# bramtoula/multi_robot_SLAM_separators

Measured on AMD Instinct MI355X. Metric: candidate keyframe-pair verifications/sec (NetVLAD NN + ORB match + RANSAC) @1/2/4/8 GPU, higher is better.
Workload: dtype u8+f16+f32+f64

## Files before the change

### multi_robot_slam_separators_amd/csrc/k_ba.hip

```cpp
#pragma once
#include "sf_device_math.hpp"
#include "sf_internal.hpp"
#include "sf_pnp_math.hpp"

namespace {

#define BA_NSUM 28

struct BaLds {
  double* X;
  double* Xc;
  float* o1;
  float* o2;
  double* red;
  double* ne_a;
  double* ne_b;
  int* misc;
};

struct BaCam {
  double fx, fy, b, info, delta;
  double R1[9], t1[3];
};

// ... 303 lines not shown
      for (int k = 0; k < 3; ++k) tt[k] = c == 0 ? cam.t1[k] : t[k];
      const double* Xi = L.X + 3 * i;
      const double Pc[3] = {((R[0] * Xi[0] + R[1] * Xi[1]) + R[2] * Xi[2]) + tt[0],
                            ((R[3] * Xi[0] + R[4] * Xi[1]) + R[5] * Xi[2]) + tt[1],
                            ((R[6] * Xi[0] + R[7] * Xi[1]) + R[8] * Xi[2]) + tt[2]};
      double r[3], J[3][3];
      const int rows = ba_edge(cam, Pc, (c == 0 ? L.o1 : L.o2) + 3 * i, r, J);
      if (rows == 0) { bad = true; continue; }
      double chi2 = r[0] * r[0] + r[1] * r[1];
      if (rows == 3) chi2 = chi2 + r[2] * r[2];
      chi2 = chi2 * cam.info;
      if (chi2 > lim) bad = true;
    }
    n_out += bad ? 1 : 0;
  }
#pragma unroll
  for (int off = 32; off >= 1; off >>= 1) n_out += __shfl_xor(n_out, off);
  __syncthreads();
  if (lane == 0) L.misc[8 + wave] = n_out;
  __syncthreads();
  n_out = L.misc[8];
#pragma unroll
  for (int w = 1; w < NW; ++w) n_out += L.misc[8 + w];

  if (tid == 0) {
    PassState o = p0;
    o.inliers = n - n_out;
    if (o.inliers < P.min_inliers) {
      o.is_null = 1;
#pragma unroll
      for (int i = 0; i < 12; ++i) o.T[i] = 0.f;
    } else {
// ... 191 lines not shown
#pragma unroll
    for (int w = 0; w < SF_BLOCK / 64; ++w) {
      const int cw = misc[4 + w];
      if (w < wave) woff += cw;
      total += cw;
    }
    if (ok) {
      const int k = n_ba + woff + before;
      pts[k] = make_float4(ax, ay, az, 0.f);
      cidx[k] = c;
      ones[k] = 1;
    }
    n_ba += total;
    __syncthreads();
  }
#pragma unroll
  for (int off = 32; off >= 1; off >>= 1) { uni += __shfl_xor(uni, off); uni_m += __shfl_xor(uni_m, off); }
  if (lane == 0) { atomicAdd(&misc[0], uni); atomicAdd(&misc[1], uni_m); }
  __syncthreads();
  uni = misc[0];
  uni_m = misc[1];
  if (tid == 0) {
    PassState a = fwd[pair];
    const PassState b = back[pair];
    a.matches = PNP ? uni_m : (a.matches > b.matches ? a.matches : b.matches);
    const bool adjust = P.bundle_adjustment != 0 && !a.is_null && n_ba > 0;
    misc[2] = adjust ? 1 : 0;
    if (adjust) {
      a.inliers = n_ba;
    } else {
      a.inliers = uni;
      if (!b.is_null) {
// ... 58 lines not shown
```

### multi_robot_slam_separators_amd/csrc/k_guided.hip

```cpp
#include "sf_device_math.hpp"
#include "sf_internal.hpp"

namespace {

#define GUIDED_CPT 8
#define GUIDED_CAND_CAP (GUIDED_CPT * 256)
#define GUIDED_CAND_CAP_NARROW 1216


__device__ __forceinline__ bool guided_eligible(const PassState& p1, const DeviceParams& P, const int4& mF, int Kf, int Kt,
                                                PassState& pass2_out, uint8_t& guided_flag_out, CorrHeader& hdr_out) {
  bool ident = true;
#pragma unroll
  for (int i = 0; i < 12; ++i) ident = ident && (p1.T[i] == ((i == 0 || i == 5 || i == 10) ? 1.f : 0.f));
  const bool eligible = !p1.is_null && !ident && P.guess_win > 0 && mF.y > 0 && P.calibrated && Kf > 0 && Kt > 0;
  if (!eligible && threadIdx.x == 0) {
    pass2_out = p1;
    guided_flag_out = 0;
    CorrHeader h = {0, 0, 0, 0};
    hdr_out = h;
  }
  return eligible;
}

// ... 54 lines not shown
    __syncthreads();
    int woff = 0, total = 0;
#pragma unroll
    for (int w = 0; w < NW; ++w) {
      int c = misc[4 + w];
      if (w < wave) woff += c;
      total += c;
    }
    if (flag) out[running + woff + before] = (uint32_t)i | ((uint32_t)m << 16);
    running += total;
    __syncthreads();
  }
  return running;
}

__device__ __forceinline__ void guided_sum_counts(int& n_finite, int& n_proj, int* misc) {
  for (int off = 32; off >= 1; off >>= 1) {
    n_finite += __shfl_xor(n_finite, off);
    n_proj += __shfl_xor(n_proj, off);
  }
  if ((threadIdx.x & 63) == 0) {
    atomicAdd(&misc[0], n_finite);
    atomicAdd(&misc[1], n_proj);
  }
  __syncthreads();
  n_finite = misc[0];
  n_proj = misc[1];
}

template <int NW>
__device__ __forceinline__ bool guided_finish(const StoreView& st, int pair, int sT, const int4& mT, int Kt,
                                              const float* xF, int n_finite, int n_proj, int n_corr, const uint32_t* out,
                                              PassState& pass2_out, uint8_t& guided_flag_out, CorrHeader& hdr_out,
                                              int32_t* __restrict__ list, int32_t* __restrict__ counter,
// ... 132 lines not shown
    for (int j = 0; j < 2; ++j) {
      const int t = base + tid + j * NT;
      if (t < Kt) {
        raw[t] = k2[j];
        const int cidx = cell_of(k2[j]);
        if (cidx >= 0) atomicAdd(&cell_start[cidx + 1], 1);
      }
    }
  }
  __syncthreads();
  {
    const int per = (NC + NT - 1) / NT;
    const int c0 = tid * per, c1 = min(c0 + per, NC);
    int local = 0;
    for (int cidx = c0; cidx < c1; ++cidx) local += cell_start[cidx + 1];
    int incl = local;
    for (int off = 1; off < 64; off <<= 1) {
      const int o = __shfl_up(incl, off);
      if (lane >= off) incl += o;
    }
    if (lane == 63) misc[8 + wave] = incl;
    __syncthreads();
    int woff = 0;
    for (int w = 0; w < wave; ++w) woff += misc[8 + w];
    int run = woff + incl - local;
    __syncthreads();
    for (int cidx = c0; cidx < c1; ++cidx) {
      const int cnt_c = cell_start[cidx + 1];
      cell_start[cidx + 1] = run + cnt_c;
      run += cnt_c;
    }
  }
  __syncthreads();
  for (int t = tid; t < Kt; t += NT) {
    const float4 k = raw[t];
// ... 76 lines not shown
                nb = 0;
              }
              const uint32_t rec = ((uint32_t)i << 16) | (uint32_t)t;
              hb0 = nb == 0 ? rec : hb0; hb1 = nb == 1 ? rec : hb1; hb2 = nb == 2 ? rec : hb2; hb3 = nb == 3 ? rec : hb3;
              ++nb;
              ++oi;
              if (last < 0 || t > last) last = t;
            }
          }
        }
      }
    }
#ifdef SF_CHAIN_TRACE
    if (base == 0 && wave == 0 && P.dbg_trace) {
      int mx = dbg_trips, sm = dbg_entries;
      for (int off = 32; off >= 1; off >>= 1) { mx = max(mx, __shfl_xor(mx, off)); sm += __shfl_xor(sm, off); }
      if (lane == 0) P.dbg_trace[(size_t)pair * SF_TRACE_SLOTS + 31] = ((unsigned long long)mx << 32) | (unsigned)sm;
    }
#endif
    if (base == 0) SF_TRACE_MARK(P, pair, 29);
    {
      int incl = nb;
#pragma unroll
      for (int off = 1; off < 64; off <<= 1) {
        const int o = __shfl_up(incl, off);
        if (lane >= off) incl += o;
      }
      const int wtot = __shfl(incl, 63);
      int wbase = 0;
      if (wtot > 0) {
        if (lane == 0) wbase = atomicAdd(&misc[3], wtot);
        wbase = __shfl(wbase, 0);
        const int s0 = wbase + incl - nb;
        if (s0 + nb <= cand_cap) {
          if (nb > 0) cand[s0] = hb0;
          if (nb > 1) cand[s0 + 1] = hb1;
          if (nb > 2) cand[s0 + 2] = hb2;
          if (nb > 3) cand[s0 + 3] = hb3;
        }
      }
    }
    if (base == 0) SF_TRACE_MARK(P, pair, 30);
#ifndef SF_CHAIN_TRACE
// ... 6 lines not shown
    }
#endif
    if (i < Kf) {
      oilast[i] = ((uint32_t)min(oi, 0xFFFF) << 16) | (uint32_t)(last & 0xFFFF);
      key1[i] = 0xFFFFFFFFu;
      key2[i] = 0xFFFFFFFFu;
    }
  }
  __syncthreads();
  SF_TRACE_MARK(P, pair, 24);
  const int n_cand = misc[3];
#ifndef SF_CHAIN_TRACE
  if (P.dbg_trace) {
    int mine = 0;
    for (int i = tid; i < Kf; i += NT) mine += (int)(oilast[i] >> 16);
    for (int off = 32; off >= 1; off >>= 1) mine += __shfl_xor(mine, off);
    if (lane == 0) atomicAdd(&misc[12], mine);
    __syncthreads();
    if (tid == 0 && misc[12] != n_cand) atomicAdd(&P.dbg_trace[2], 1ull);
    __syncthreads();
  }
#endif
#ifdef SF_CHAIN_TRACE
  if (tid == 0 && P.dbg_trace) P.dbg_trace[(size_t)pair * SF_TRACE_SLOTS + 27] = (unsigned long long)n_cand;
#endif
  if (!L2 && n_cand <= cand_cap) {
    if constexpr (NW == 4) {
    uint32_t ck[GUIDED_CPT], ci[GUIDED_CPT];
#pragma unroll
    for (int j = 0; j < GUIDED_CPT; ++j) {
      const int c = tid + j * NT;
// ... 304 lines not shown
          b0 = min(b0, key);
        }
        ++oi;
        one = i;
      }
    }
    int m = -1;
    if (oi >= 2) {
      if constexpr (L2) { if (i0 >= 0 && f0 < P.nndr * f1) m = i0; }
      else if ((float)(b0 >> 16) < P.nndr * (float)(b1 >> 16)) m = (int)(b0 & 0xFFFFu);
    } else if (oi == 1) {
      m = one;
    }
    if (m >= 0 && atomicCAS(&claimw[m], EMPTY, (uint32_t)t) != EMPTY) atomicOr(&claimw[m], SHARED);
  }
  guided_sum_counts(n_finite, n_proj, misc);
  const int n_corr = guided_compact<NW>(Kf, out, misc, [&](int i) {
    const uint32_t w = claimw[i];
    return (w & SHARED) ? -1 : (int)w;
  });
  return guided_finish<NW>(st, pair, sT, mT, Kt, xF, n_finite, n_proj, n_corr, out, pass2_out, guided_flag_out, hdr_out,
                           list, counter, P, misc);
}

template <int W, bool L2 = false>
__global__ void __launch_bounds__(SF_BLOCK)
k_guided_tp(StoreView st, const int32_t* __restrict__ pair_from, const int32_t* __restrict__ pair_to,
            const PassState* __restrict__ pass1, PassState* __restrict__ pass2, uint8_t* __restrict__ guided_flag,
            uint32_t* __restrict__ corr, CorrHeader* __restrict__ hdr, int32_t* __restrict__ list,
            int32_t* __restrict__ counter, DeviceParams P) {
  extern __shared__ __attribute__((aligned(16))) int smem[];
// ... 162 lines not shown
```

### multi_robot_slam_separators_amd/csrc/k_pnp.hip

```cpp
#include "sf_device_math.hpp"
#include "sf_internal.hpp"
#include "sf_pnp_math.hpp"
#include "k_ba.hip"

namespace {

#define PNP_NSUM 28

__host__ __device__ inline size_t sf_pnp_lds_bytes_dev(int kcap, int iterations, bool bear = true, int nw = 4) {
  (void)iterations;
  return (size_t)kcap * (16 + (bear ? 24 : 0) + 8 + 4 + 4 + 4 + 2) + 128 * 8 + 64 * 4 + 16 * 4 + 12 * 64 * 4 +
         (size_t)(nw + 1) * 64 * 4 + 16 * 4 + 2 * 32 * 8;
}

struct PnpLds {
  float4* obj;
  float2* img;
  double* bear;
  uint32_t* cidx;
  float* e1;
  float* e2;
  uint8_t* mask;
  uint8_t* mask_b;
  int* counts;
  double* red;
  int* misc;
  float* hyp;
  int* hyp_cnt;
  float* best;
  double* ne_a;
  double* ne_b;
};

template <int NW = 4>
__device__ __forceinline__ int block_sum_i(int v, int* misc, int tid) {
  const int lane = tid & 63, wave = tid >> 6;
#pragma unroll
  for (int off = 32; off >= 1; off >>= 1) v += __shfl_xor(v, off);
  __syncthreads();
  if (lane == 0) misc[8 + wave] = v;
  __syncthreads();
  int t = misc[8];
#pragma unroll
  for (int w = 1; w < NW; ++w) t += misc[8 + w];
  return t;
}

struct PnpCam {
  double fx, fy;
  float fxf, fyf, thr2f;
};

__device__ __forceinline__ bool pnp_inlier(const PnpLds& L, const PnpCam& cam, const float (&c)[12], int i) {
// ... 33 lines not shown
      const double inv = 1.0 / sqrt((un * un + vn * vn) + 1.0);
      f[k][0] = un * inv; f[k][1] = vn * inv; f[k][2] = inv;
    }
  }
  const float4 p4 = L.obj[s3];
  const float2 o4 = L.img[s3];
  const double P4[3] = {(double)p4.x, (double)p4.y, (double)p4.z};
  return sfd::p3p_best(P, f, P4, (double)o4.x, (double)o4.y, cam.fx, cam.fy, coef);
}

template <int NW>
__device__ inline void pnp_normal_eq(const PnpLds& L, const PnpCam& cam, int m, const uint8_t* mask,
                                     const double (&q)[4], const double (&t)[3], double* out, int tid) {
  double R[9];
  sfd::quat_to_R(q, R);
  sfd::canon_reduce_to_lds<PNP_NSUM, 32, NW>(m, tid, L.red, out, [&](int i, double (&ne)[PNP_NSUM]) {
    if (!mask[i]) return;
    const float4 p = L.obj[i];
    const float2 o = L.img[i];
    const double Px = (double)p.x, Py = (double)p.y, Pz = (double)p.z;
    const double Yx = (R[0] * Px + R[1] * Py) + R[2] * Pz;
    const double Yy = (R[3] * Px + R[4] * Py) + R[5] * Pz;
    const double Yz = (R[6] * Px + R[7] * Py) + R[8] * Pz;
    const double X = Yx + t[0], Y = Yy + t[1], Z = Yz + t[2];
    if (Z > 0.0) {
      const double iz = 1.0 / Z;
      const double xn = X * iz, yn = Y * iz;
      const double ru = cam.fx * xn - (double)o.x;
      const double rv = cam.fy * yn - (double)o.y;
      const double a0 = cam.fx * iz, a2 = -(a0 * xn);
      const double b1 = cam.fy * iz, b2 = -(b1 * yn);
// ... 382 lines not shown
    int n_sizes = 0, z1 = 0, z2 = 0, z3 = 0, z4 = 0;
    do {
      pnp_lm<NW>(L, cam, m, prev, q, t, tid);
      z4 = z3; z3 = z2; z2 = z1; z1 = n_prev;
      ++n_sizes;
      __syncthreads();
      n_new = pnp_select<NW>(L, cam, m, q, t, error_threshold, neu, tid);
      if (n_new < min_count) {
        ++refine_iterations;
        if (refine_iterations >= P.pnp_refine_iterations) break;
        continue;
      }
      double s1[1] = {0.0};
      if constexpr (NW == 4) {
        for (int i = tid; i < m; i += NT) if (neu[i]) s1[0] += (double)L.e1[i];
        sfd::block_sum_canon<1, 32>(s1, L.red, tid);
      } else {
        sfd::canon_reduce<1, 32, NW>(m, tid, L.red, s1, [&](int i, double (&a)[1]) { if (neu[i]) a[0] += (double)L.e1[i]; });
      }
      const float mean = (float)(s1[0] / (double)n_new);
      float variance = 0.0f;
      if (n_new > 1) {
        double s2[1] = {0.0};
        if constexpr (NW == 4) {
          for (int i = tid; i < m; i += NT) {
            if (neu[i]) { const float dlt = L.e1[i] - mean; s2[0] += (double)(dlt * dlt); }
          }
          sfd::block_sum_canon<1, 32>(s2, L.red, tid);
        } else {
          sfd::canon_reduce<1, 32, NW>(m, tid, L.red, s2, [&](int i, double (&a)[1]) {
            if (neu[i]) { const float dlt = L.e1[i] - mean; a[0] += (double)(dlt * dlt); }
          });
        }
        variance = (float)(s2[0] / (double)(n_new - 1));
      }
      const float sthr = (float)P.refine_sigma * sqrtf(variance);
      error_threshold = sthr < inlier_thr ? sthr : inlier_thr;
      inlier_changed = false;
      { uint8_t* tp = prev; prev = neu; neu = tp; const int tn = n_prev; n_prev = n_new; n_new = tn; }
      if (n_new != n_prev) {
        if (n_sizes >= 4 && z1 == z3 && z2 == z4) break;
        inlier_changed = true;
        continue;
// ... 122 lines not shown
  const bool guided = guided_flag != nullptr && guided_flag[pair] != 0;
  const bool g0 = sf_pnp_dir_gate(0, h, st.meta[sF].x, guided, min_inliers);
  const bool g1 = sf_pnp_dir_gate(1, h, st.meta[sF].x, guided, min_inliers);
  const float* xF = st.xyz + (size_t)sF * kcap * 3;
  const float* xT = st.xyz + (size_t)sT * kcap * 3;
  const uint32_t* cl = corr + (size_t)pair * kcap;
  int uni = 0, uni_m = 0;
  for (int i = lane; i < kcap; i += 64) uni += (mask_f[(size_t)pair * kcap + i] | mask_b[(size_t)pair * kcap + i]) ? 1 : 0;
  for (int i = lane; i < h.n_corr; i += 64) {
    const uint32_t c = cl[i];
    bool m = false;
    if (g0) { const float* a = xF + 3 * (c & 0xFFFFu); m = sfd::finite3(a[0], a[1], a[2]); }
    if (g1 && !m) { const float* b = xT + 3 * (c >> 16); m = sfd::finite3(b[0], b[1], b[2]); }
    uni_m += m ? 1 : 0;
  }
#pragma unroll
  for (int off = 32; off >= 1; off >>= 1) { uni += __shfl_xor(uni, off); uni_m += __shfl_xor(uni_m, off); }
  if (lane != 0) return;
  PassState a = fwd[pair];
  const PassState b = back[pair];
  a.inliers = uni;
  a.matches = uni_m;
  if (!b.is_null) {
    float inv[12];
    sfd::rigid_inverse_canon(b.T, inv);
    if (a.is_null) {
#pragma unroll
      for (int i = 0; i < 12; ++i) a.T[i] = inv[i];
      a.is_null = 0;
      a.var = b.var;
      a.var_ang = b.var_ang;
    } else {
// ... 78 lines not shown
```

### multi_robot_slam_separators_amd/csrc/k_ransac.hip

```cpp
#include "sf_device_math.hpp"
#include "sf_internal.hpp"
#include "k_ba.hip"

namespace {

struct RansacLds {
  float4* src;
  float4* dst;
  float* d2;
  uint8_t* mask_a;
  uint8_t* mask_b;
  double* red;
  unsigned long long* sums;
  int* misc;
  float* hyp;
  int* hyp_cnt;
  float* best;
  float* bc;
  uint32_t* cidx;
};

__device__ __forceinline__ RansacLds ransac_carve(unsigned char* p, int kcap) {
  RansacLds L;
  L.src = (float4*)p; p += (size_t)kcap * 16;
// ... 113 lines not shown
  for (int i = tid; i < m4; i += 64 * NW) {
    float r2 = __int_as_float(0x7F800000);
    if (i < m) {
      float4 p = L.src[i], q = L.dst[i];
      const float v = sfd::residual2(coef, p.x, p.y, p.z, q.x, q.y, q.z);
      const bool in = (double)v < thr2;
      r2 = in ? v : r2;
      const bool was = prev ? prev[i] != 0 : false;
      mask[i] = in ? 1 : 0;
      const bool low = in && !(thr < sigma * sqrt(2.1981 * (double)v));
      acc += (in ? 1ull : 0ull) + (low ? (1ull << 13) : 0ull) + ((was != in) ? (1ull << 26) : 0ull);
    }
    L.d2[i] = r2;
  }
  const int lane = tid & 63, wave = tid >> 6;
#pragma unroll
  for (int off = 32; off >= 1; off >>= 1) acc += __shfl_xor(acc, off);
  __syncthreads();
  if (lane == 0) L.sums[wave] = acc;
  __syncthreads();
  unsigned long long t = L.sums[0];
#pragma unroll
  for (int w = 1; w < NW; ++w) t += L.sums[w];
  SelCounts c;
  c.n = (int)(t & 0x1FFFull);
  c.low = (int)((t >> 13) & 0x1FFFull);
  c.diff = (int)((t >> 26) & 0x1FFFull);
  return c;
}

typedef __attribute__((address_space(3))) const float* lds_cfloat_p;
typedef __attribute__((address_space(3))) unsigned* lds_uint_p;
// ... 6 lines not shown
  __syncthreads();
  unsigned prefix = 0u;
#pragma unroll 1
  for (int p = 0; p < 4; ++p) {
    const int shift = 24 - 8 * p;
    for (int i = tid; i < m4; i += NT) {
      const unsigned bits = __float_as_uint(d2[i]);
      if (p == 0 || (bits >> (shift + 8)) == prefix)
        __hip_atomic_fetch_add(&hist[p * 256 + ((bits >> shift) & 255u)], 1u, __ATOMIC_RELAXED, __HIP_MEMORY_SCOPE_WORKGROUP);
    }
    __syncthreads();
    if (wave == 0) {
      const unsigned h0 = hist[p * 256 + 4 * lane], h1 = hist[p * 256 + 4 * lane + 1], h2 = hist[p * 256 + 4 * lane + 2],
                     h3 = hist[p * 256 + 4 * lane + 3];
      const unsigned s = (h0 + h1) + (h2 + h3);
      unsigned incl = s;
#pragma unroll
      for (int off = 1; off < 64; off <<= 1) {
        const unsigned y = __shfl_up(incl, off);
        if (lane >= off) incl += y;
      }
      const unsigned excl = incl - s;
      if (excl <= (unsigned)rank && (unsigned)rank < incl) {
        unsigned r = (unsigned)rank - excl;
        int b = 0;
        if (r >= h0) { r -= h0; b = 1; if (r >= h1) { r -= h1; b = 2; if (r >= h2) { r -= h2; b = 3; } } }
        misc[2] = (int)((prefix << 8) | (unsigned)(4 * lane + b));
        misc[3] = (int)r;
      }
    }
    __syncthreads();
    prefix = (unsigned)misc[2];
    rank = misc[3];
  }
  return __uint_as_float(prefix);
}
// ... 49 lines not shown
  if (i < m) {
    const float4 p = L.src[i], q = L.dst[i];
    const float r2 = sfd::residual2(coef, p.x, p.y, p.z, q.x, q.y, q.z);
    cnt += (r2 <= thr2f) ? 1 : 0;
  }
  return cnt;
}

struct ScanState {
  int best;
  int best_it;
  int it;
  double k;
};

__device__ __forceinline__ int shfl_up_from(int v, int off, int lane) {
  const int src = lane >= off ? lane - off : lane;
  return __builtin_amdgcn_ds_bpermute(src << 2, v);
}
__device__ __forceinline__ double shfl_up_from(double v, int off, int lane) {
  const int src = lane >= off ? lane - off : lane;
  const long long b = __double_as_longlong(v);
  const int lo = __builtin_amdgcn_ds_bpermute(src << 2, (int)(b & 0xFFFFFFFFll));
  const int hi = __builtin_amdgcn_ds_bpermute(src << 2, (int)(b >> 32));
  return __longlong_as_double(((long long)hi << 32) | (unsigned)lo);
}

__device__ __forceinline__ bool replay_round(const RansacLds& L, ScanState& S, int base, int R, int lane, int c,
                                             bool present, int max_it, bool adaptive, double inv_m,
                                             double log_probability, bool park = true) {
  int x = present ? c : -1;
#pragma unroll
  for (int off = 1; off < 64; off <<= 1) {
    const int y = shfl_up_from(x, off, lane);
    if (lane >= off) x = max(x, y);
  }
  x = max(x, S.best);
  double kj = 1.0;
  if (x >= 0) {
    const double w = (double)x * inv_m;
    double pno = 1.0 - (w * w) * w;
    if (pno < 2.220446049250313e-16) pno = 2.220446049250313e-16;
    if (pno > 1.0 - 2.220446049250313e-16) pno = 1.0 - 2.220446049250313e-16;
    kj = log_probability / sfd::canon_log(pno);
  }
  double kprev = shfl_up_from(kj, 1, lane);
  if (lane == 0) kprev = S.k;
  const int it = base + lane;
  const bool top_ok = present && (!adaptive || (double)it < kprev) && c >= 0;
  const unsigned long long fail = ~__ballot(top_ok);
  const int n_proc = fail ? (__ffsll((long long)fail) - 1) : 64;
// ... 376 lines not shown
  extern __shared__ __attribute__((aligned(16))) unsigned char smem_raw[];
  const int pair = list[blockIdx.x];
  ransac_body<DIR>(st, pair, pair_from[pair], pair_to[pair], corr + (size_t)pair * st.kcap, hdr[pair].n_corr,
                       pass[pair], P, smem_raw, 2, mask ? mask + (size_t)pair * st.kcap : nullptr);
  if (extra_3dof && threadIdx.x == 0) pass_to3dof(pass[pair], extra_3dof);
}

__global__ void __launch_bounds__(64)
k_merge_directions(const int32_t* __restrict__ list, const int32_t* __restrict__ counter, PassState* __restrict__ fwd,
                   const PassState* __restrict__ back, const uint8_t* __restrict__ mask_f,
                   const uint8_t* __restrict__ mask_b, int kcap, int extra_3dof) {
  if ((int)blockIdx.x >= *counter) return;
  const int pair = list[blockIdx.x], lane = threadIdx.x;
  int uni = 0;
  for (int i = lane; i < kcap; i += 64) uni += (mask_f[(size_t)pair * kcap + i] | mask_b[(size_t)pair * kcap + i]) ? 1 : 0;
#pragma unroll
  for (int off = 32; off >= 1; off >>= 1) uni += __shfl_xor(uni, off);
  if (lane != 0) return;
  PassState a = fwd[pair];
  const PassState b = back[pair];
  a.inliers = uni;
  a.matches = a.matches > b.matches ? a.matches : b.matches;
  if (!b.is_null) {
    float inv[12];
    sfd::rigid_inverse_canon(b.T, inv);
    if (a.is_null) {
#pragma unroll
      for (int i = 0; i < 12; ++i) a.T[i] = inv[i];
      a.is_null = 0;
      a.var = b.var;
      a.var_ang = b.var_ang;
    } else {
// ... 77 lines not shown
```

### multi_robot_slam_separators_amd/csrc/sf_device_math.hpp

```cpp
#pragma once
#include <hip/hip_runtime.h>
#include <stdint.h>

namespace sfd {

__device__ __forceinline__ uint64_t mix64(uint64_t z) {
  z += 0x9E3779B97F4A7C15ULL;
  z = (z ^ (z >> 30)) * 0xBF58476D1CE4E5B9ULL;
  z = (z ^ (z >> 27)) * 0x94D049BB133111EBULL;
  return z ^ (z >> 31);
}

__device__ __forceinline__ void sample_triplet(uint64_t seed, uint32_t it, uint32_t attempt, uint32_t m,
                                               uint32_t& i0, uint32_t& i1, uint32_t& i2) {
  uint64_t ha = mix64(seed ^ mix64(((uint64_t)it << 32) | (uint64_t)attempt));
  uint64_t hb = mix64(ha);
  uint32_t r0 = (uint32_t)(ha >> 32), r1 = (uint32_t)ha, r2 = (uint32_t)(hb >> 32);
  i0 = __umulhi(r0, m);
  i1 = __umulhi(r1, m - 1);
  if (i1 >= i0) ++i1;
  i2 = __umulhi(r2, m - 2);
  uint32_t lo = i0 < i1 ? i0 : i1, hi = i0 < i1 ? i1 : i0;
  if (i2 >= lo) ++i2;
  if (i2 >= hi) ++i2;
// ... 198 lines not shown
    coef[4 * j + 2] = (float)R[3 * j + 2];
    coef[4 * j + 3] = (float)t;
  }
}

__device__ __forceinline__ float residual2(const float (&c)[12], float px, float py, float pz,
                                           float qx, float qy, float qz) {
  float tx = __fmaf_rn(c[2], pz, __fmaf_rn(c[1], py, __fmaf_rn(c[0], px, c[3])));
  float ty = __fmaf_rn(c[6], pz, __fmaf_rn(c[5], py, __fmaf_rn(c[4], px, c[7])));
  float tz = __fmaf_rn(c[10], pz, __fmaf_rn(c[9], py, __fmaf_rn(c[8], px, c[11])));
  float dx = tx - qx, dy = ty - qy, dz = tz - qz;
  return __fmaf_rn(dz, dz, __fmaf_rn(dy, dy, dx * dx));
}


template <int C>
__device__ __forceinline__ void sum_stage(double (&w)[32], int& idx, int lane, int off) {
  if constexpr (C > 1) {
    const bool up = (lane & off) != 0;
#pragma unroll
    for (int k = 0; k < C / 2; ++k) {
      const double send = up ? w[k] : w[k + C / 2];
      const double keep = up ? w[k + C / 2] : w[k];
      w[k] = keep + __shfl_xor(send, off);
    }
    idx += up ? C / 2 : 0;
  } else {
    w[0] = w[0] + __shfl_xor(w[0], off);
  }
}

template <int N, int STRIDE>
__device__ __forceinline__ void block_sum_canon(double (&v)[N], double* red, int tid) {
  static_assert(N >= 1 && N <= 32 && STRIDE >= N, "at most 32 values");
  constexpr int P = N <= 1 ? 1 : N <= 2 ? 2 : N <= 4 ? 4 : N <= 8 ? 8 : N <= 16 ? 16 : 32;
  static_assert(STRIDE >= P, "scratch rows must hold the padded count");
  const int lane = tid & 63, wave = tid >> 6;
  double w[32];
#pragma unroll
  for (int k = 0; k < 32; ++k) w[k] = k < N ? v[k] : 0.0;
  int idx = 0;
  sum_stage<P>(w, idx, lane, 32);
  sum_stage<(P / 2 > 1 ? P / 2 : 1)>(w, idx, lane, 16);
  sum_stage<(P / 4 > 1 ? P / 4 : 1)>(w, idx, lane, 8);
  sum_stage<(P / 8 > 1 ? P / 8 : 1)>(w, idx, lane, 4);
  sum_stage<(P / 16 > 1 ? P / 16 : 1)>(w, idx, lane, 2);
  sum_stage<(P / 32 > 1 ? P / 32 : 1)>(w, idx, lane, 1);
  __syncthreads();
  red[wave * STRIDE + idx] = w[0];
  __syncthreads();
#pragma unroll
  for (int k = 0; k < N; ++k) v[k] = ((red[k] + red[STRIDE + k]) + red[2 * STRIDE + k]) + red[3 * STRIDE + k];
}

template <int N, int STRIDE, int NW, class F>
__device__ __forceinline__ void canon_reduce(int m, int tid, double* red, double (&out)[N], F acc) {
  if constexpr (NW == 4) {
#pragma unroll
    for (int k = 0; k < N; ++k) out[k] = 0.0;
    for (int i = tid; i < m; i += 256) acc(i, out);
    block_sum_canon<N, STRIDE>(out, red, tid);
  } else {
    static_assert(NW == 1 || NW == 2, "one, two or four wavefronts");
    constexpr int P = N <= 1 ? 1 : N <= 2 ? 2 : N <= 4 ? 4 : N <= 8 ? 8 : N <= 16 ? 16 : 32;
    static_assert(STRIDE >= P, "scratch rows must hold the padded count");
    const int lane = tid & 63, wave = tid >> 6;
    __syncthreads();
#pragma unroll 1
    for (int j = 0; j < 4 / NW; ++j) {
      const int vw = wave * (4 / NW) + j;
      if (64 * vw >= m) {
        if (lane < P) red[vw * STRIDE + lane] = 0.0;
        continue;
      }
      double w[32];
#pragma unroll
      for (int k = 0; k < 32; ++k) w[k] = 0.0;
      {
        double v[N];
#pragma unroll
        for (int k = 0; k < N; ++k) v[k] = 0.0;
        for (int i = lane + 64 * vw; i < m; i += 256) acc(i, v);
#pragma unroll
        for (int k = 0; k < N; ++k) w[k] = v[k];
      }
      int idx = 0;
      sum_stage<P>(w, idx, lane, 32);
      sum_stage<(P / 2 > 1 ? P / 2 : 1)>(w, idx, lane, 16);
      sum_stage<(P / 4 > 1 ? P / 4 : 1)>(w, idx, lane, 8);
      sum_stage<(P / 8 > 1 ? P / 8 : 1)>(w, idx, lane, 4);
      sum_stage<(P / 16 > 1 ? P / 16 : 1)>(w, idx, lane, 2);
      sum_stage<(P / 32 > 1 ? P / 32 : 1)>(w, idx, lane, 1);
      red[vw * STRIDE + idx] = w[0];
    }
    __syncthreads();
#pragma unroll
    for (int k = 0; k < N; ++k) out[k] = ((red[k] + red[STRIDE + k]) + red[2 * STRIDE + k]) + red[3 * STRIDE + k];
  }
}

template <int N, int STRIDE>
__device__ __forceinline__ void block_sum_canon_to_lds(const double (&v)[N], double* red, double* out, int tid) {
  static_assert(N >= 1 && N <= 32 && STRIDE >= N, "at most 32 values");
  constexpr int P = N <= 1 ? 1 : N <= 2 ? 2 : N <= 4 ? 4 : N <= 8 ? 8 : N <= 16 ? 16 : 32;
  static_assert(STRIDE >= P, "scratch rows must hold the padded count");
  const int lane = tid & 63, wave = tid >> 6;
  double w[32];
#pragma unroll
  for (int k = 0; k < 32; ++k) w[k] = k < N ? v[k] : 0.0;
  int idx = 0;
  sum_stage<P>(w, idx, lane, 32);
  sum_stage<(P / 2 > 1 ? P / 2 : 1)>(w, idx, lane, 16);
  sum_stage<(P / 4 > 1 ? P / 4 : 1)>(w, idx, lane, 8);
  sum_stage<(P / 8 > 1 ? P / 8 : 1)>(w, idx, lane, 4);
  sum_stage<(P / 16 > 1 ? P / 16 : 1)>(w, idx, lane, 2);
  sum_stage<(P / 32 > 1 ? P / 32 : 1)>(w, idx, lane, 1);
  __syncthreads();
  red[wave * STRIDE + idx] = w[0];
  __syncthreads();
  if (tid < N) out[tid] = ((red[tid] + red[STRIDE + tid]) + red[2 * STRIDE + tid]) + red[3 * STRIDE + tid];
  __syncthreads();
}

template <int N, int STRIDE, int NW, bool ONCE = false, class F>
__device__ __forceinline__ void canon_reduce_to_lds(int m, int tid, double* red, double* out, F acc) {
  if constexpr (NW == 4) {
    double v[N];
#pragma unroll
    for (int k = 0; k < N; ++k) v[k] = 0.0;
    if constexpr (ONCE) { if (tid < m) acc(tid, v); }
    else { for (int i = tid; i < m; i += 256) acc(i, v); }
    block_sum_canon_to_lds<N, STRIDE>(v, red, out, tid);
  } else {
    static_assert(NW == 1 || NW == 2, "one, two or four wavefronts");
    constexpr int P = N <= 1 ? 1 : N <= 2 ? 2 : N <= 4 ? 4 : N <= 8 ? 8 : N <= 16 ? 16 : 32;
    static_assert(STRIDE >= P, "scratch rows must hold the padded count");
    const int lane = tid & 63, wave = tid >> 6;
    __syncthreads();
#pragma unroll 1
    for (int j = 0; j < 4 / NW; ++j) {
      const int vw = wave * (4 / NW) + j;
      if (64 * vw >= m) {
        if (lane < P) red[vw * STRIDE + lane] = 0.0;
        continue;
      }
      double w[32];
#pragma unroll
      for (int k = 0; k < 32; ++k) w[k] = 0.0;
      {
        double v[N];
#pragma unroll
        for (int k = 0; k < N; ++k) v[k] = 0.0;
        if constexpr (ONCE) { if (lane + 64 * vw < m) acc(lane + 64 * vw, v); }
        else { for (int i = lane + 64 * vw; i < m; i += 256) acc(i, v); }
#pragma unroll
        for (int k = 0; k < N; ++k) w[k] = v[k];
      }
      int idx = 0;
      sum_stage<P>(w, idx, lane, 32);
      sum_stage<(P / 2 > 1 ? P / 2 : 1)>(w, idx, lane, 16);
      sum_stage<(P / 4 > 1 ? P / 4 : 1)>(w, idx, lane, 8);
      sum_stage<(P / 8 > 1 ? P / 8 : 1)>(w, idx, lane, 4);
      sum_stage<(P / 16 > 1 ? P / 16 : 1)>(w, idx, lane, 2);
      sum_stage<(P / 32 > 1 ? P / 32 : 1)>(w, idx, lane, 1);
      red[vw * STRIDE + idx] = w[0];
    }
    __syncthreads();
    if (tid < N) out[tid] = ((red[tid] + red[STRIDE + tid]) + red[2 * STRIDE + tid]) + red[3 * STRIDE + tid];
    __syncthreads();
  }
}

__device__ __forceinline__ bool finite3(float x, float y, float z) {
  return isfinite(x) && isfinite(y) && isfinite(z);
}

__device__ inline void to3dof_canon(float* T) {
  const double r11 = (double)T[0], r21 = (double)T[4];
  const double h = sqrt(r11 * r11 + r21 * r21);
// ... 71 lines not shown
```

Before: 24.47 million.

## Replace shuffle-based wave reductions and scans with DPP and permlane swap intrinsics

Adds DPP-based wave_sum, wave_max, wave_scan_add and wave_scan_max helpers, plus permlane16/32 swap primitives, and routes most wave reductions and prefix scans across BA, guided matching, PnP and RANSAC kernels through them. The canonical double-precision block reductions get a lane-swap path that replaces ds_bpermute shuffles with DPP and permlane swaps, and skip accumulation in wavefronts with no work. The aim is lower cross-lane latency and LDS traffic in reduction-heavy inner loops. Some call sites keep the old shuffle path to preserve bitwise summation order, and the new lane-swap ordering must match the old canonical order for results to stay deterministic.

```diff
diff --git a/multi_robot_slam_separators_amd/csrc/k_ba.hip b/multi_robot_slam_separators_amd/csrc/k_ba.hip
--- a/multi_robot_slam_separators_amd/csrc/k_ba.hip
+++ b/multi_robot_slam_separators_amd/csrc/k_ba.hip
@@ -341,8 +341,7 @@
     }
     n_out += bad ? 1 : 0;
   }
-#pragma unroll
-  for (int off = 32; off >= 1; off >>= 1) n_out += __shfl_xor(n_out, off);
+  n_out = sfd::wave_sum(n_out);
   __syncthreads();
   if (lane == 0) L.misc[8 + wave] = n_out;
   __syncthreads();
@@ -564,8 +563,7 @@
     n_ba += total;
     __syncthreads();
   }
-#pragma unroll
-  for (int off = 32; off >= 1; off >>= 1) { uni += __shfl_xor(uni, off); uni_m += __shfl_xor(uni_m, off); }
+  uni = sfd::wave_sum(uni); uni_m = sfd::wave_sum(uni_m);
   if (lane == 0) { atomicAdd(&misc[0], uni); atomicAdd(&misc[1], uni_m); }
   __syncthreads();
   uni = misc[0];
diff --git a/multi_robot_slam_separators_amd/csrc/k_guided.hip b/multi_robot_slam_separators_amd/csrc/k_guided.hip
--- a/multi_robot_slam_separators_amd/csrc/k_guided.hip
+++ b/multi_robot_slam_separators_amd/csrc/k_guided.hip
@@ -92,10 +92,16 @@
   return running;
 }
 
+template <bool LANES = true>
 __device__ __forceinline__ void guided_sum_counts(int& n_finite, int& n_proj, int* misc) {
-  for (int off = 32; off >= 1; off >>= 1) {
-    n_finite += __shfl_xor(n_finite, off);
-    n_proj += __shfl_xor(n_proj, off);
+  if constexpr (LANES) {
+    n_finite = sfd::wave_sum(n_finite);
+    n_proj = sfd::wave_sum(n_proj);
+  } else {
+    for (int off = 32; off >= 1; off >>= 1) {
+      n_finite += __shfl_xor(n_finite, off);
+      n_proj += __shfl_xor(n_proj, off);
+    }
   }
   if ((threadIdx.x & 63) == 0) {
     atomicAdd(&misc[0], n_finite);
@@ -258,11 +264,7 @@
     const int c0 = tid * per, c1 = min(c0 + per, NC);
     int local = 0;
     for (int cidx = c0; cidx < c1; ++cidx) local += cell_start[cidx + 1];
-    int incl = local;
-    for (int off = 1; off < 64; off <<= 1) {
-      const int o = __shfl_up(incl, off);
-      if (lane >= off) incl += o;
-    }
+    const int incl = sfd::wave_scan_add(local);
     if (lane == 63) misc[8 + wave] = incl;
     __syncthreads();
     int woff = 0;
@@ -369,19 +371,14 @@
 #ifdef SF_CHAIN_TRACE
     if (base == 0 && wave == 0 && P.dbg_trace) {
       int mx = dbg_trips, sm = dbg_entries;
-      for (int off = 32; off >= 1; off >>= 1) { mx = max(mx, __shfl_xor(mx, off)); sm += __shfl_xor(sm, off); }
+      mx = sfd::wave_max(mx); sm = sfd::wave_sum(sm);
       if (lane == 0) P.dbg_trace[(size_t)pair * SF_TRACE_SLOTS + 31] = ((unsigned long long)mx << 32) | (unsigned)sm;
     }
 #endif
     if (base == 0) SF_TRACE_MARK(P, pair, 29);
     {
-      int incl = nb;
-#pragma unroll
-      for (int off = 1; off < 64; off <<= 1) {
-        const int o = __shfl_up(incl, off);
-        if (lane >= off) incl += o;
-      }
-      const int wtot = __shfl(incl, 63);
+      const int incl = sfd::wave_scan_add(nb);
+      const int wtot = __builtin_amdgcn_readlane(incl, 63);
       int wbase = 0;
       if (wtot > 0) {
         if (lane == 0) wbase = atomicAdd(&misc[3], wtot);
@@ -418,7 +415,7 @@
   if (P.dbg_trace) {
     int mine = 0;
     for (int i = tid; i < Kf; i += NT) mine += (int)(oilast[i] >> 16);
-    for (int off = 32; off >= 1; off >>= 1) mine += __shfl_xor(mine, off);
+    mine = sfd::wave_sum(mine);
     if (lane == 0) atomicAdd(&misc[12], mine);
     __syncthreads();
     if (tid == 0 && misc[12] != n_cand) atomicAdd(&P.dbg_trace[2], 1ull);
@@ -753,7 +750,7 @@
     }
     if (m >= 0 && atomicCAS(&claimw[m], EMPTY, (uint32_t)t) != EMPTY) atomicOr(&claimw[m], SHARED);
   }
-  guided_sum_counts(n_finite, n_proj, misc);
+  guided_sum_counts<false>(n_finite, n_proj, misc);
   const int n_corr = guided_compact<NW>(Kf, out, misc, [&](int i) {
     const uint32_t w = claimw[i];
     return (w & SHARED) ? -1 : (int)w;
diff --git a/multi_robot_slam_separators_amd/csrc/k_pnp.hip b/multi_robot_slam_separators_amd/csrc/k_pnp.hip
--- a/multi_robot_slam_separators_amd/csrc/k_pnp.hip
+++ b/multi_robot_slam_separators_amd/csrc/k_pnp.hip
@@ -32,11 +32,13 @@
   double* ne_b;
 };
 
+template <int NW>
+constexpr bool PNP_SUM_LANES = SF_SUM_LANES != 0 && NW != 4;
+
 template <int NW = 4>
 __device__ __forceinline__ int block_sum_i(int v, int* misc, int tid) {
   const int lane = tid & 63, wave = tid >> 6;
-#pragma unroll
-  for (int off = 32; off >= 1; off >>= 1) v += __shfl_xor(v, off);
+  v = sfd::wave_sum(v);
   __syncthreads();
   if (lane == 0) misc[8 + wave] = v;
   __syncthreads();
@@ -100,7 +102,7 @@
                                      const double (&q)[4], const double (&t)[3], double* out, int tid) {
   double R[9];
   sfd::quat_to_R(q, R);
-  sfd::canon_reduce_to_lds<PNP_NSUM, 32, NW>(m, tid, L.red, out, [&](int i, double (&ne)[PNP_NSUM]) {
+  sfd::canon_reduce_to_lds<PNP_NSUM, 32, NW, false, PNP_SUM_LANES<NW>>(m, tid, L.red, out, [&](int i, double (&ne)[PNP_NSUM]) {
     if (!mask[i]) return;
     const float4 p = L.obj[i];
     const float2 o = L.img[i];
@@ -513,7 +515,7 @@
       double s1[1] = {0.0};
       if constexpr (NW == 4) {
         for (int i = tid; i < m; i += NT) if (neu[i]) s1[0] += (double)L.e1[i];
-        sfd::block_sum_canon<1, 32>(s1, L.red, tid);
+        sfd::block_sum_canon<1, 32, PNP_SUM_LANES<NW>>(s1, L.red, tid);
       } else {
         sfd::canon_reduce<1, 32, NW>(m, tid, L.red, s1, [&](int i, double (&a)[1]) { if (neu[i]) a[0] += (double)L.e1[i]; });
       }
@@ -525,7 +527,7 @@
           for (int i = tid; i < m; i += NT) {
             if (neu[i]) { const float dlt = L.e1[i] - mean; s2[0] += (double)(dlt * dlt); }
           }
-          sfd::block_sum_canon<1, 32>(s2, L.red, tid);
+          sfd::block_sum_canon<1, 32, PNP_SUM_LANES<NW>>(s2, L.red, tid);
         } else {
           sfd::canon_reduce<1, 32, NW>(m, tid, L.red, s2, [&](int i, double (&a)[1]) {
             if (neu[i]) { const float dlt = L.e1[i] - mean; a[0] += (double)(dlt * dlt); }
@@ -678,8 +680,7 @@
     if (g1 && !m) { const float* b = xT + 3 * (c >> 16); m = sfd::finite3(b[0], b[1], b[2]); }
     uni_m += m ? 1 : 0;
   }
-#pragma unroll
-  for (int off = 32; off >= 1; off >>= 1) { uni += __shfl_xor(uni, off); uni_m += __shfl_xor(uni_m, off); }
+  uni = sfd::wave_sum(uni); uni_m = sfd::wave_sum(uni_m);
   if (lane != 0) return;
   PassState a = fwd[pair];
   const PassState b = back[pair];
diff --git a/multi_robot_slam_separators_amd/csrc/k_ransac.hip b/multi_robot_slam_separators_amd/csrc/k_ransac.hip
--- a/multi_robot_slam_separators_amd/csrc/k_ransac.hip
+++ b/multi_robot_slam_separators_amd/csrc/k_ransac.hip
@@ -151,8 +151,7 @@
     L.d2[i] = r2;
   }
   const int lane = tid & 63, wave = tid >> 6;
-#pragma unroll
-  for (int off = 32; off >= 1; off >>= 1) acc += __shfl_xor(acc, off);
+  acc = sfd::wave_sum(acc);
   __syncthreads();
   if (lane == 0) L.sums[wave] = acc;
   __syncthreads();
@@ -189,12 +188,7 @@
       const unsigned h0 = hist[p * 256 + 4 * lane], h1 = hist[p * 256 + 4 * lane + 1], h2 = hist[p * 256 + 4 * lane + 2],
                      h3 = hist[p * 256 + 4 * lane + 3];
       const unsigned s = (h0 + h1) + (h2 + h3);
-      unsigned incl = s;
-#pragma unroll
-      for (int off = 1; off < 64; off <<= 1) {
-        const unsigned y = __shfl_up(incl, off);
-        if (lane >= off) incl += y;
-      }
+      const unsigned incl = (unsigned)sfd::wave_scan_add((int)s);
       const unsigned excl = incl - s;
       if (excl <= (unsigned)rank && (unsigned)rank < incl) {
         unsigned r = (unsigned)rank - excl;
@@ -274,10 +268,6 @@
   double k;
 };
 
-__device__ __forceinline__ int shfl_up_from(int v, int off, int lane) {
-  const int src = lane >= off ? lane - off : lane;
-  return __builtin_amdgcn_ds_bpermute(src << 2, v);
-}
 __device__ __forceinline__ double shfl_up_from(double v, int off, int lane) {
   const int src = lane >= off ? lane - off : lane;
   const long long b = __double_as_longlong(v);
@@ -289,12 +279,7 @@
 __device__ __forceinline__ bool replay_round(const RansacLds& L, ScanState& S, int base, int R, int lane, int c,
                                              bool present, int max_it, bool adaptive, double inv_m,
                                              double log_probability, bool park = true) {
-  int x = present ? c : -1;
-#pragma unroll
-  for (int off = 1; off < 64; off <<= 1) {
-    const int y = shfl_up_from(x, off, lane);
-    if (lane >= off) x = max(x, y);
-  }
+  int x = sfd::wave_scan_max(present ? c : -1);
   x = max(x, S.best);
   double kj = 1.0;
   if (x >= 0) {
@@ -701,8 +686,7 @@
   const int pair = list[blockIdx.x], lane = threadIdx.x;
   int uni = 0;
   for (int i = lane; i < kcap; i += 64) uni += (mask_f[(size_t)pair * kcap + i] | mask_b[(size_t)pair * kcap + i]) ? 1 : 0;
-#pragma unroll
-  for (int off = 32; off >= 1; off >>= 1) uni += __shfl_xor(uni, off);
+  uni = sfd::wave_sum(uni);
   if (lane != 0) return;
   PassState a = fwd[pair];
   const PassState b = back[pair];
diff --git a/multi_robot_slam_separators_amd/csrc/sf_device_math.hpp b/multi_robot_slam_separators_amd/csrc/sf_device_math.hpp
--- a/multi_robot_slam_separators_amd/csrc/sf_device_math.hpp
+++ b/multi_robot_slam_separators_amd/csrc/sf_device_math.hpp
@@ -236,52 +236,199 @@
 }
 
 
-template <int C>
-__device__ __forceinline__ void sum_stage(double (&w)[32], int& idx, int lane, int off) {
-  if constexpr (C > 1) {
-    const bool up = (lane & off) != 0;
-#pragma unroll
-    for (int k = 0; k < C / 2; ++k) {
-      const double send = up ? w[k] : w[k + C / 2];
-      const double keep = up ? w[k + C / 2] : w[k];
-      w[k] = keep + __shfl_xor(send, off);
-    }
-    idx += up ? C / 2 : 0;
+#define SF_DPP_QUAD_XOR1 0xB1
+#define SF_DPP_QUAD_XOR2 0x4E
+#define SF_DPP_ROW_SHL4 0x104
+#define SF_DPP_ROW_SHR1 0x111
+#define SF_DPP_ROW_SHR2 0x112
+#define SF_DPP_ROW_SHR4 0x114
+#define SF_DPP_ROW_SHR8 0x118
+#define SF_DPP_ROW_ROR8 0x128
+#define SF_DPP_ROW_MIRROR 0x140
+#define SF_DPP_ROW_HALF_MIRROR 0x141
+#define SF_DPP_ROW_BCAST15 0x142
+#define SF_DPP_ROW_BCAST31 0x143
+
+template <int OFF>
+__device__ __forceinline__ int lane_xor_dpp(int x) {
+  static_assert(OFF == 1 || OFF == 2 || OFF == 4 || OFF == 8, "a lane distance inside a row of 16");
+  if constexpr (OFF == 1) return __builtin_amdgcn_mov_dpp(x, SF_DPP_QUAD_XOR1, 0xf, 0xf, false);
+  else if constexpr (OFF == 2) return __builtin_amdgcn_mov_dpp(x, SF_DPP_QUAD_XOR2, 0xf, 0xf, false);
+  else if constexpr (OFF == 8) return __builtin_amdgcn_mov_dpp(x, SF_DPP_ROW_ROR8, 0xf, 0xf, false);
+  else {
+    const int t = __builtin_amdgcn_mov_dpp(x, SF_DPP_ROW_SHL4, 0xf, 0x5, false);
+    return __builtin_amdgcn_update_dpp(t, x, SF_DPP_ROW_SHR4, 0xf, 0xa, false);
+  }
+}
+template <int OFF>
+__device__ __forceinline__ double lane_xor_dpp(double x) {
+  return __hiloint2double(lane_xor_dpp<OFF>(__double2hiint(x)), lane_xor_dpp<OFF>(__double2loint(x)));
+}
+
+template <int OFF>
+__device__ __forceinline__ void lane_swap(unsigned& a, unsigned& b) {
+  static_assert(OFF == 16 || OFF == 32, "the two swap distances");
+  if constexpr (OFF == 32) {
+    const auto r = __builtin_amdgcn_permlane32_swap(a, b, false, false);
+    a = r[0]; b = r[1];
   } else {
-    w[0] = w[0] + __shfl_xor(w[0], off);
-  }
-}
-
-template <int N, int STRIDE>
-__device__ __forceinline__ void block_sum_canon(double (&v)[N], double* red, int tid) {
+    const auto r = __builtin_amdgcn_permlane16_swap(a, b, false, false);
+    a = r[0]; b = r[1];
+  }
+}
+template <int OFF>
+__device__ __forceinline__ void lane_swap(double& a, double& b) {
+  unsigned al = (unsigned)__double2loint(a), ah = (unsigned)__double2hiint(a);
+  unsigned bl = (unsigned)__double2loint(b), bh = (unsigned)__double2hiint(b);
+  lane_swap<OFF>(al, bl);
+  lane_swap<OFF>(ah, bh);
+  a = __hiloint2double((int)ah, (int)al);
+  b = __hiloint2double((int)bh, (int)bl);
+}
+
+__device__ __forceinline__ int wave_scan_add(int v) {
+  v += __builtin_amdgcn_update_dpp(0, v, SF_DPP_ROW_SHR1, 0xf, 0xf, false);
+  v += __builtin_amdgcn_update_dpp(0, v, SF_DPP_ROW_SHR2, 0xf, 0xf, false);
+  v += __builtin_amdgcn_update_dpp(0, v, SF_DPP_ROW_SHR4, 0xf, 0xf, false);
+  v += __builtin_amdgcn_update_dpp(0, v, SF_DPP_ROW_SHR8, 0xf, 0xf, false);
+  v += __builtin_amdgcn_update_dpp(0, v, SF_DPP_ROW_BCAST15, 0xa, 0xf, false);
+  v += __builtin_amdgcn_update_dpp(0, v, SF_DPP_ROW_BCAST31, 0xc, 0xf, false);
+  return v;
+}
+__device__ __forceinline__ int wave_scan_max(int v) {
+  v = max(v, __builtin_amdgcn_update_dpp(v, v, SF_DPP_ROW_SHR1, 0xf, 0xf, false));
+  v = max(v, __builtin_amdgcn_update_dpp(v, v, SF_DPP_ROW_SHR2, 0xf, 0xf, false));
+  v = max(v, __builtin_amdgcn_update_dpp(v, v, SF_DPP_ROW_SHR4, 0xf, 0xf, false));
+  v = max(v, __builtin_amdgcn_update_dpp(v, v, SF_DPP_ROW_SHR8, 0xf, 0xf, false));
+  v = max(v, __builtin_amdgcn_update_dpp(v, v, SF_DPP_ROW_BCAST15, 0xa, 0xf, false));
+  v = max(v, __builtin_amdgcn_update_dpp(v, v, SF_DPP_ROW_BCAST31, 0xc, 0xf, false));
+  return v;
+}
+
+template <class OP>
+__device__ __forceinline__ int wave_reduce_i(int v, OP op) {
+  v = op(v, __builtin_amdgcn_mov_dpp(v, SF_DPP_QUAD_XOR1, 0xf, 0xf, false));
+  v = op(v, __builtin_amdgcn_mov_dpp(v, SF_DPP_QUAD_XOR2, 0xf, 0xf, false));
+  v = op(v, __builtin_amdgcn_mov_dpp(v, SF_DPP_ROW_HALF_MIRROR, 0xf, 0xf, false));
+  v = op(v, __builtin_amdgcn_mov_dpp(v, SF_DPP_ROW_MIRROR, 0xf, 0xf, false));
+  unsigned a = (unsigned)v, b = (unsigned)v;
+  lane_swap<16>(a, b);
+  v = op((int)a, (int)b);
+  a = (unsigned)v; b = (unsigned)v;
+  lane_swap<32>(a, b);
+  return op((int)a, (int)b);
+}
+__device__ __forceinline__ int wave_sum(int v) { return wave_reduce_i(v, [](int x, int y) { return x + y; }); }
+__device__ __forceinline__ int wave_max(int v) { return wave_reduce_i(v, [](int x, int y) { return max(x, y); }); }
+template <int CTRL>
+__device__ __forceinline__ unsigned long long dpp_mov64(unsigned long long x) {
+  const unsigned lo = (unsigned)__builtin_amdgcn_mov_dpp((int)(unsigned)x, CTRL, 0xf, 0xf, false);
+  const unsigned hi = (unsigned)__builtin_amdgcn_mov_dpp((int)(unsigned)(x >> 32), CTRL, 0xf, 0xf, false);
+  return ((unsigned long long)hi << 32) | lo;
+}
+template <int OFF>
+__device__ __forceinline__ unsigned long long swap_sum64(unsigned long long v) {
+  unsigned al = (unsigned)v, ah = (unsigned)(v >> 32), bl = al, bh = ah;
+  lane_swap<OFF>(al, bl);
+  lane_swap<OFF>(ah, bh);
+  return (((unsigned long long)ah << 32) | al) + (((unsigned long long)bh << 32) | bl);
+}
+__device__ __forceinline__ unsigned long long wave_sum(unsigned long long v) {
+  v += dpp_mov64<SF_DPP_QUAD_XOR1>(v);
+  v += dpp_mov64<SF_DPP_QUAD_XOR2>(v);
+  v += dpp_mov64<SF_DPP_ROW_HALF_MIRROR>(v);
+  v += dpp_mov64<SF_DPP_ROW_MIRROR>(v);
+  v = swap_sum64<16>(v);
+  return swap_sum64<32>(v);
+}
+
+#ifndef SF_SUM_LANES
+#define SF_SUM_LANES 1
+#endif
+template <int C, int OFF, bool LANES>
+__device__ __forceinline__ void sum_stage(double (&w)[32], int& idx, int lane) {
+  if constexpr (!LANES) {
+    if constexpr (C > 1) {
+      const bool up = (lane & OFF) != 0;
+#pragma unroll
+      for (int k = 0; k < C / 2; ++k) {
+        const double send = up ? w[k] : w[k + C / 2];
+        const double keep = up ? w[k + C / 2] : w[k];
+        w[k] = keep + __shfl_xor(send, OFF);
+      }
+      idx += up ? C / 2 : 0;
+    } else {
+      w[0] = w[0] + __shfl_xor(w[0], OFF);
+    }
+  } else if constexpr (OFF >= 16) {
+    if constexpr (C > 1) {
+#pragma unroll
+      for (int k = 0; k < C / 2; ++k) {
+        double a = w[k], b = w[k + C / 2];
+        lane_swap<OFF>(a, b);
+        w[k] = a + b;
+      }
+      idx += (lane & OFF) ? C / 2 : 0;
+    } else {
+      double a = w[0], b = w[0];
+      lane_swap<OFF>(a, b);
+      w[0] = a + b;
+    }
+  } else {
+    if constexpr (C > 1) {
+      const bool up = (lane & OFF) != 0;
+#pragma unroll
+      for (int k = 0; k < C / 2; ++k) {
+        const double send = up ? w[k] : w[k + C / 2];
+        const double keep = up ? w[k + C / 2] : w[k];
+        w[k] = keep + lane_xor_dpp<OFF>(send);
+      }
+      idx += up ? C / 2 : 0;
+    } else {
+      w[0] = w[0] + lane_xor_dpp<OFF>(w[0]);
+    }
+  }
+}
+
+template <int P, bool LANES>
+__device__ __forceinline__ void sum_stages(double (&w)[32], int& idx, int lane) {
+  sum_stage<P, 32, LANES>(w, idx, lane);
+  sum_stage<(P / 2 > 1 ? P / 2 : 1), 16, LANES>(w, idx, lane);
+  sum_stage<(P / 4 > 1 ? P / 4 : 1), 8, LANES>(w, idx, lane);
+  sum_stage<(P / 8 > 1 ? P / 8 : 1), 4, LANES>(w, idx, lane);
+  sum_stage<(P / 16 > 1 ? P / 16 : 1), 2, LANES>(w, idx, lane);
+  sum_stage<(P / 32 > 1 ? P / 32 : 1), 1, LANES>(w, idx, lane);
+}
+
+template <int N, int STRIDE, bool LANES = (SF_SUM_LANES != 0)>
+__device__ __forceinline__ void block_sum_canon(double (&v)[N], double* red, int tid, bool live = true) {
   static_assert(N >= 1 && N <= 32 && STRIDE >= N, "at most 32 values");
   constexpr int P = N <= 1 ? 1 : N <= 2 ? 2 : N <= 4 ? 4 : N <= 8 ? 8 : N <= 16 ? 16 : 32;
   static_assert(STRIDE >= P, "scratch rows must hold the padded count");
   const int lane = tid & 63, wave = tid >> 6;
   double w[32];
-#pragma unroll
-  for (int k = 0; k < 32; ++k) w[k] = k < N ? v[k] : 0.0;
   int idx = 0;
-  sum_stage<P>(w, idx, lane, 32);
-  sum_stage<(P / 2 > 1 ? P / 2 : 1)>(w, idx, lane, 16);
-  sum_stage<(P / 4 > 1 ? P / 4 : 1)>(w, idx, lane, 8);
-  sum_stage<(P / 8 > 1 ? P / 8 : 1)>(w, idx, lane, 4);
-  sum_stage<(P / 16 > 1 ? P / 16 : 1)>(w, idx, lane, 2);
-  sum_stage<(P / 32 > 1 ? P / 32 : 1)>(w, idx, lane, 1);
+  if (live) {
+#pragma unroll
+    for (int k = 0; k < 32; ++k) w[k] = k < N ? v[k] : 0.0;
+    sum_stages<P, LANES>(w, idx, lane);
+  }
   __syncthreads();
-  red[wave * STRIDE + idx] = w[0];
+  if (live) red[wave * STRIDE + idx] = w[0];
+  else if (lane < P) red[wave * STRIDE + lane] = 0.0;
   __syncthreads();
 #pragma unroll
   for (int k = 0; k < N; ++k) v[k] = ((red[k] + red[STRIDE + k]) + red[2 * STRIDE + k]) + red[3 * STRIDE + k];
 }
 
-template <int N, int STRIDE, int NW, class F>
+template <int N, int STRIDE, int NW, bool LANES = (SF_SUM_LANES != 0), class F>
 __device__ __forceinline__ void canon_reduce(int m, int tid, double* red, double (&out)[N], F acc) {
   if constexpr (NW == 4) {
+    const bool live = 64 * (tid >> 6) < m;
 #pragma unroll
     for (int k = 0; k < N; ++k) out[k] = 0.0;
-    for (int i = tid; i < m; i += 256) acc(i, out);
-    block_sum_canon<N, STRIDE>(out, red, tid);
+    if (live) for (int i = tid; i < m; i += 256) acc(i, out);
+    block_sum_canon<N, STRIDE, LANES>(out, red, tid, live);
   } else {
     static_assert(NW == 1 || NW == 2, "one, two or four wavefronts");
     constexpr int P = N <= 1 ? 1 : N <= 2 ? 2 : N <= 4 ? 4 : N <= 8 ? 8 : N <= 16 ? 16 : 32;
@@ -307,12 +454,7 @@
         for (int k = 0; k < N; ++k) w[k] = v[k];
       }
       int idx = 0;
-      sum_stage<P>(w, idx, lane, 32);
-      sum_stage<(P / 2 > 1 ? P / 2 : 1)>(w, idx, lane, 16);
-      sum_stage<(P / 4 > 1 ? P / 4 : 1)>(w, idx, lane, 8);
-      sum_stage<(P / 8 > 1 ? P / 8 : 1)>(w, idx, lane, 4);
-      sum_stage<(P / 16 > 1 ? P / 16 : 1)>(w, idx, lane, 2);
-      sum_stage<(P / 32 > 1 ? P / 32 : 1)>(w, idx, lane, 1);
+      sum_stages<P, LANES>(w, idx, lane);
       red[vw * STRIDE + idx] = w[0];
     }
     __syncthreads();
@@ -321,38 +463,40 @@
   }
 }
 
-template <int N, int STRIDE>
-__device__ __forceinline__ void block_sum_canon_to_lds(const double (&v)[N], double* red, double* out, int tid) {
+template <int N, int STRIDE, bool LANES = (SF_SUM_LANES != 0)>
+__device__ __forceinline__ void block_sum_canon_to_lds(const double (&v)[N], double* red, double* out, int tid,
+                                                       bool live = true) {
   static_assert(N >= 1 && N <= 32 && STRIDE >= N, "at most 32 values");
   constexpr int P = N <= 1 ? 1 : N <= 2 ? 2 : N <= 4 ? 4 : N <= 8 ? 8 : N <= 16 ? 16 : 32;
   static_assert(STRIDE >= P, "scratch rows must hold the padded count");
   const int lane = tid & 63, wave = tid >> 6;
   double w[32];
-#pragma unroll
-  for (int k = 0; k < 32; ++k) w[k] = k < N ? v[k] : 0.0;
   int idx = 0;
-  sum_stage<P>(w, idx, lane, 32);
-  sum_stage<(P / 2 > 1 ? P / 2 : 1)>(w, idx, lane, 16);
-  sum_stage<(P / 4 > 1 ? P / 4 : 1)>(w, idx, lane, 8);
-  sum_stage<(P / 8 > 1 ? P / 8 : 1)>(w, idx, lane, 4);
-  sum_stage<(P / 16 > 1 ? P / 16 : 1)>(w, idx, lane, 2);
-  sum_stage<(P / 32 > 1 ? P / 32 : 1)>(w, idx, lane, 1);
+  if (live) {
+#pragma unroll
+    for (int k = 0; k < 32; ++k) w[k] = k < N ? v[k] : 0.0;
+    sum_stages<P, LANES>(w, idx, lane);
+  }
   __syncthreads();
-  red[wave * STRIDE + idx] = w[0];
+  if (live) red[wave * STRIDE + idx] = w[0];
+  else if (lane < P) red[wave * STRIDE + lane] = 0.0;
   __syncthreads();
   if (tid < N) out[tid] = ((red[tid] + red[STRIDE + tid]) + red[2 * STRIDE + tid]) + red[3 * STRIDE + tid];
   __syncthreads();
 }
 
-template <int N, int STRIDE, int NW, bool ONCE = false, class F>
+template <int N, int STRIDE, int NW, bool ONCE = false, bool LANES = (SF_SUM_LANES != 0), class F>
 __device__ __forceinline__ void canon_reduce_to_lds(int m, int tid, double* red, double* out, F acc) {
   if constexpr (NW == 4) {
+    const bool live = 64 * (tid >> 6) < m;
     double v[N];
 #pragma unroll
     for (int k = 0; k < N; ++k) v[k] = 0.0;
-    if constexpr (ONCE) { if (tid < m) acc(tid, v); }
-    else { for (int i = tid; i < m; i += 256) acc(i, v); }
-    block_sum_canon_to_lds<N, STRIDE>(v, red, out, tid);
+    if (live) {
+      if constexpr (ONCE) { if (tid < m) acc(tid, v); }
+      else { for (int i = tid; i < m; i += 256) acc(i, v); }
+    }
+    block_sum_canon_to_lds<N, STRIDE, LANES>(v, red, out, tid, live);
   } else {
     static_assert(NW == 1 || NW == 2, "one, two or four wavefronts");
     constexpr int P = N <= 1 ? 1 : N <= 2 ? 2 : N <= 4 ? 4 : N <= 8 ? 8 : N <= 16 ? 16 : 32;
@@ -379,12 +523,7 @@
         for (int k = 0; k < N; ++k) w[k] = v[k];
       }
       int idx = 0;
-      sum_stage<P>(w, idx, lane, 32);
-      sum_stage<(P / 2 > 1 ? P / 2 : 1)>(w, idx, lane, 16);
-      sum_stage<(P / 4 > 1 ? P / 4 : 1)>(w, idx, lane, 8);
-      sum_stage<(P / 8 > 1 ? P / 8 : 1)>(w, idx, lane, 4);
-      sum_stage<(P / 16 > 1 ? P / 16 : 1)>(w, idx, lane, 2);
-      sum_stage<(P / 32 > 1 ? P / 32 : 1)>(w, idx, lane, 1);
+      sum_stages<P, LANES>(w, idx, lane);
       red[vw * STRIDE + idx] = w[0];
     }
     __syncthreads();
```

After: 25.12 million, median of 6. +2.7%, better.
